# lior1990/hp-vae-gan

Measured on AMD Instinct MI355X. Metric: train iters/sec per pyramid scale, air_balloons 13f@144p, higher is better.
Workload: dtype f32

## Files before the change

### hp-vae-gan_amd/csrc/conv_mfma.hip

```cpp
#include "hpvg_common.h"
#include "hpvg_host.h"
#include "hpvg.h"
#include <stdlib.h>

namespace {

__device__ const float g_zero_word[16] = {0.f, 0.f, 0.f, 0.f, 0.f, 0.f, 0.f, 0.f, 0.f, 0.f, 0.f, 0.f, 0.f, 0.f, 0.f, 0.f};
constexpr long HPVG_ZERO_PLANE_FLOATS = 1L << 18;
__device__ float g_zero_plane[HPVG_ZERO_PLANE_FLOATS];

#ifdef HPVG_TRACE
__device__ unsigned long long g_trace[8192 * 4];
__device__ unsigned long long g_phase[8192 * 4];
#define HPVG_PH(i) { unsigned long long now_ = __builtin_readcyclecounter(); ph_a[i] += now_ - ph_t; ph_t = now_; }
#define HPVG_PH_INIT unsigned long long ph_t = __builtin_readcyclecounter(); unsigned long long ph_a[4] = {0, 0, 0, 0};
#define HPVG_PH_END if (threadIdx.x == 0) { for (int i_ = 0; i_ < 4; ++i_) g_phase[4 * blockIdx.x + i_] = ph_a[i_]; }
#define HPVG_TRACE_BEGIN unsigned long long tr_t0 = wall_clock64(); unsigned long long tr_c0 = __builtin_readcyclecounter();
#define HPVG_TRACE_END                                                              \
  if (threadIdx.x == 0 && blockIdx.x + gridDim.x * (blockIdx.y + gridDim.y * blockIdx.z) < 8192) { \
    unsigned long long* tr = g_trace + 4 * (blockIdx.x + gridDim.x * (blockIdx.y + gridDim.y * blockIdx.z)); \
    tr[0] = tr_t0;                                                                  \
    tr[1] = wall_clock64();                                                         \
    tr[2] = __builtin_amdgcn_s_getreg((31 << 11) | 4);                              \
    tr[3] = (__builtin_amdgcn_s_getreg((31 << 11) | 20) & 0xF) | ((__builtin_readcyclecounter() - tr_c0) << 8); \
// ... 675 lines not shown
      if (n < CO9) {
#pragma unroll
        for (int jj = 0; jj < JB; ++jj)
#pragma unroll
          for (int e = 0; e < 16; ++e) P[n * pitch + GP * grp + JB * ((e & 3) + 8 * (e >> 2) + 4 * half) + jj] = acc[jj][nt][e];
      }
    }
  }
  __syncthreads();

  const int ob = g.ob[band], on = g.on[band];
  const int nout = g.Th * on;
  for (int idx = tid; idx < nout; idx += 256) {
    const int hh = idx / on, cc = idx - hh * on;
    const int gh = h0 + hh, gw = ob + cc;
    if (gh >= a.H) continue;
    const long sp = (long)t * HW + (long)gh * a.W + gw;
    for (int o = 0; o < a.Cout; ++o) {
      float v = 0.f;
#pragma unroll
      for (int dh = 0; dh < 3; ++dh)
#pragma unroll
        for (int dw = 0; dw < 3; ++dw) {
          const int gwt = gw + dw - 1;
          if (gwt >= 0 && gwt < a.W) v += P[(o * 9 + dh * 3 + dw) * pitch + (hh + dh) * RS + (gwt - wsb)];
        }
      if (a.bias) v += a.bias[o];
      if (a.out_lrelu) v = hpvg_lrelu(v);
      a.y[((long)b * a.Cout + o) * a.T * HW + sp] = v;
    }
  }
}

__global__ void conv_pack_narrow_kernel(const float* __restrict__ w, const float* __restrict__ inv_scale, float* __restrict__ wn,
                                        int Cin_k, int Cout_k, int KT, int NT, int ksteps, int transpose_flip, long total) {
  const long idx = (long)blockIdx.x * blockDim.x + threadIdx.x;
  if (idx >= total) return;
  const int lane = idx & 63;
  long r = idx >> 6;
  const int nt = r % NT;
  const int s = (int)(r / NT);
  const int k = (lane >> 5) * ksteps + s;
  const int n = nt * 32 + (lane & 31);
  const int c = k / KT, dt = k - c * KT;
  const int o = n / 9, tap = dt * 9 + (n - o * 9);
  const int taps = KT * 9;
  float val = 0.f;
  if (o < Cout_k && c < Cin_k) {
    if (!transpose_flip) val = w[((long)o * Cin_k + c) * taps + tap];
    else val = w[((long)c * Cout_k + o) * taps + (taps - 1 - tap)];
    if (inv_scale) val *= inv_scale[0];
  }
  wn[idx] = val;
}

__global__ void conv_pack_kernel(const float* __restrict__ w, const float* __restrict__ inv_scale, float* __restrict__ wp,
                                 int Cin_k, int Cout_k, int taps, int CC, int nchunk, int mbtot, int transpose_flip,
                                 long total_direct, long total) {
  const long idx = (long)blockIdx.x * blockDim.x + threadIdx.x;
  if (idx >= total) return;
  if (idx >= total_direct) {
    const long iw = idx - total_direct;
    const long nw1 = ((long)((Cin_k + WINO_CC - 1) / WINO_CC) * (taps / 9) * 3 * 4 + 4) * mbtot * 64 * (WINO_CC / 2);
    float val = iw < nw1 ? wino_pack_value(w, iw, Cin_k, Cout_k, taps / 9, (Cin_k + WINO_CC - 1) / WINO_CC, mbtot, transpose_flip)
                         : wino2_pack_value(w, iw - nw1, Cin_k, Cout_k, (Cin_k + 3) / 4, 2 * ((mbtot + 1) / 2), transpose_flip);
    if (inv_scale) val *= inv_scale[0];
    wp[idx] = val;
    return;
  }
  const int CP = CC / 2;
  long r = idx;
  const int cp = r % CP; r /= CP;
  const int lane = r % 64; r /= 64;
  const int mb = r % mbtot; r /= mbtot;
  const int tap = r % taps; r /= taps;
  const int ch = (int)r;
  float val = 0.f;
  if (ch < nchunk) {
    const int o = mb * 32 + (lane & 31);
    const int c = ch * CC + 2 * cp + (lane >> 5);
    if (o < Cout_k && c < Cin_k) {
      if (!transpose_flip) val = w[((long)o * Cin_k + c) * taps + tap];
      else val = w[((long)c * Cout_k + o) * taps + (taps - 1 - tap)];
      if (inv_scale) val *= inv_scale[0];
    }
  }
  wp[idx] = val;
}

struct PackBatchArgs {
  const float* w[HPVG_PACK_BATCH_MAX];
  float* wp[HPVG_PACK_BATCH_MAX];
  int flip[HPVG_PACK_BATCH_MAX];
};
__global__ void conv_pack_batch_kernel(const PackBatchArgs a, int C, int taps, int CC, int nchunk, int mbtot, long total_direct,
                                       long total) {
  const long idx = (long)blockIdx.x * blockDim.x + threadIdx.x;
  if (idx >= total) return;
  const int it = blockIdx.y;
  const float* __restrict__ w = a.w[it];
  const int transpose_flip = a.flip[it];
  if (idx >= total_direct) {
    const long iw = idx - total_direct;
    const long nw1 = ((long)((C + WINO_CC - 1) / WINO_CC) * (taps / 9) * 3 * 4 + 4) * mbtot * 64 * (WINO_CC / 2);
    a.wp[it][idx] = iw < nw1 ? wino_pack_value(w, iw, C, C, taps / 9, (C + WINO_CC - 1) / WINO_CC, mbtot, transpose_flip)
                             : wino2_pack_value(w, iw - nw1, C, C, (C + 3) / 4, 2 * ((mbtot + 1) / 2), transpose_flip);
    return;
  }
  const int CP = CC / 2;
  long r = idx;
  const int cp = r % CP; r /= CP;
  const int lane = r % 64; r /= 64;
  const int mb = r % mbtot; r /= mbtot;
  const int tap = r % taps; r /= taps;
  const int ch = (int)r;
  float val = 0.f;
  if (ch < nchunk) {
    const int o = mb * 32 + (lane & 31);
    const int c = ch * CC + 2 * cp + (lane >> 5);
    if (o < C && c < C) {
      if (!transpose_flip) val = w[((long)o * C + c) * taps + tap];
      else val = w[((long)c * C + o) * taps + (taps - 1 - tap)];
    }
  }
  a.wp[it][idx] = val;
}

struct CShape { int B, Cin, Cout, T, H, W, KT; };
inline int conv_check(const CShape& c) {
  if (c.B < 1 || c.Cin < 1 || c.Cout < 1 || c.T < 1 || c.H < 1 || c.W < 1) return HPVG_ERR_ARG;
  return c.KT == 1 || c.KT == 3 ? HPVG_OK : HPVG_ERR_UNSUPPORTED;
}

struct CKnobs {
  bool sk_off;
  bool narrow2_off;
  bool w2r;
  bool w2d_off;
  int stagger;
  int only_nb, only_mb, only_ntw;
  int env_wino;
  int wino;
  long min_pos;
  int stg;
  int w2d;
  int gen;
};
CKnobs& cknobs() {
  static CKnobs knobs = [] {
    auto num = [](const char* name, long dflt) { const char* e = getenv(name); return e ? atol(e) : dflt; };
    CKnobs k{};
    k.sk_off = num("HPVG_CONV_SK", 1) == 0;
    k.narrow2_off = num("HPVG_NARROW2", 1) == 0;
    k.w2r = num("HPVG_WINO2R", 1) != 0;
    k.w2d_off = num("HPVG_WINO2D", 1) == 0;
    k.stagger = (int)num("HPVG_WINO_STAGGER", 0);
    k.only_nb = (int)num("HPVG_PLAN_NB", 0);
    k.only_mb = (int)num("HPVG_PLAN_MB", 0);
// ... 509 lines not shown

int pack_weight_launch(const float* w, const float* inv_scale, float* wp, int Cin_layer, int Cout_layer, int KT, int transpose_flip,
                       bool with2d, void* stream) {
  if (!w || !wp || (KT != 1 && KT != 3) || Cin_layer < 1 || Cout_layer < 1) return HPVG_ERR_ARG;
  const int Cin_k = transpose_flip ? Cout_layer : Cin_layer;
  const int Cout_k = transpose_flip ? Cin_layer : Cout_layer;
  const long total = (long)wpack_floats(Cin_k, Cout_k, KT, with2d);
  if (conv_is_narrow(Cin_k, Cout_k)) {
    hipLaunchKernelGGL(conv_pack_narrow_kernel, dim3(hpvg_cdiv(total, 256)), dim3(256), 0, (hipStream_t)stream, w, inv_scale, wp,
                       Cin_k, Cout_k, KT, hpvg_cdiv(9 * Cout_k, 32), hpvg_cdiv(Cin_k * KT, 2), transpose_flip, total);
    return hpvg_launch_status();
  }
  const int CC = conv_cc(Cin_k);
  hipLaunchKernelGGL(conv_pack_kernel, dim3(hpvg_cdiv(total, 256)), dim3(256), 0, (hipStream_t)stream, w, inv_scale, wp, Cin_k, Cout_k,
                     KT * 9, CC, hpvg_cdiv(Cin_k, CC), hpvg_cdiv(Cout_k, 32), transpose_flip, (long)direct_pack_floats(Cin_k, Cout_k, KT),
                     total);
  return hpvg_launch_status();
}

int pack_batch_launch(int n, const float* const* w, float* const* wp, const int* flip, int C, int KT, bool with2d, void* stream) {
  if (n < 1 || n > HPVG_PACK_BATCH_MAX || !w || !wp || !flip || C <= 4 || (KT != 1 && KT != 3)) return HPVG_ERR_ARG;
  PackBatchArgs a;
  for (int i = 0; i < n; ++i) {
    if (!w[i] || !wp[i]) return HPVG_ERR_ARG;
    a.w[i] = w[i]; a.wp[i] = wp[i]; a.flip[i] = flip[i];
  }
  const int CC = conv_cc(C);
  const long total = (long)wpack_floats(C, C, KT, with2d);
  hipLaunchKernelGGL(conv_pack_batch_kernel, dim3(hpvg_cdiv(total, 256), n), dim3(256), 0, (hipStream_t)stream, a, C, KT * 9, CC,
                     hpvg_cdiv(C, CC), hpvg_cdiv(C, 32), (long)direct_pack_floats(C, C, KT), total);
  return hpvg_launch_status();
}

int write_plan(const Plan& p, int out4, int ntiles, int* out) {
  out[0] = p.L; out[1] = p.Tw; out[2] = p.nrange; out[3] = p.ntw; out[4] = out4; out[5] = p.NB; out[6] = p.MB;
  out[7] = p.gridy; out[8] = (int)p.lds; out[9] = ntiles;
  return HPVG_OK;
}

}

extern "C" {

size_t hpvg_conv_wpack_floats(int Cin, int Cout, int KT) { return wpack_floats(Cin, Cout, KT, true); }
size_t hpvg_conv_wpack_floats_for(int Cin, int Cout, int KT, int B, int T, int H, int W) {
  return wpack_floats(Cin, Cout, KT, wants_wino2d({B, Cin, Cout, T, H, W, KT}));
}
int hpvg_conv_wants_wino2d(int B, int Cin, int Cout, int T, int H, int W, int KT) { return wants_wino2d({B, Cin, Cout, T, H, W, KT}) ? 1 : 0; }

int hpvg_conv_pack_weight_f32(const float* w, const float* inv_scale, float* wp, int Cin_layer, int Cout_layer, int KT,
                              int transpose_flip, void* stream) {
  return pack_weight_launch(w, inv_scale, wp, Cin_layer, Cout_layer, KT, transpose_flip, true, stream);
}
int hpvg_conv_pack_weight_for_f32(const float* w, const float* inv_scale, float* wp, int Cin_layer, int Cout_layer, int KT,
                                  int transpose_flip, int B, int T, int H, int W, void* stream) {
  const int Cin_k = transpose_flip ? Cout_layer : Cin_layer, Cout_k = transpose_flip ? Cin_layer : Cout_layer;
  return pack_weight_launch(w, inv_scale, wp, Cin_layer, Cout_layer, KT, transpose_flip, wants_wino2d({B, Cin_k, Cout_k, T, H, W, KT}), stream);
}
int hpvg_conv_pack_weight_batch_f32(int n, const float* const* w, float* const* wp, const int* flip, int C, int KT, void* stream) {
  return pack_batch_launch(n, w, wp, flip, C, KT, true, stream);
}
int hpvg_conv_pack_weight_batch_for_f32(int n, const float* const* w, float* const* wp, const int* flip, int C, int KT, int B, int T,
                                        int H, int W, void* stream) {
  return pack_batch_launch(n, w, wp, flip, C, KT, wants_wino2d({B, C, C, T, H, W, KT}), stream);
}

int hpvg_conv_fwd_f32(const float* x, const float* wp, const float* bias, const float* in_scale, const float* in_shift,
                      int in_lrelu, float* y, int out_lrelu, const float* out_mask, void* ws, size_t ws_bytes, int B, int Cin,
                      int Cout, int T, int H, int W, int KT, void* stream) {
  return conv_fwd_launch({x, wp, bias, in_scale, in_shift, in_lrelu, y, out_lrelu, out_mask, nullptr, nullptr, ws, ws_bytes,
                          {B, Cin, Cout, T, H, W, KT}, (hipStream_t)stream});
}

size_t hpvg_conv_mask_words(int B, int C, int T, int H, int W) { return (size_t)B * T * H * W * hpvg_cdiv(C, 32); }

int hpvg_conv_fwd_bits_f32(const float* x, const float* wp, const float* bias, float* y, int out_lrelu, const unsigned* mask_bits,
                           unsigned* bits_out, void* ws, size_t ws_bytes, int B, int Cin, int Cout, int T, int H, int W, int KT,
                           void* stream) {
  if (conv_is_narrow(Cin, Cout)) return HPVG_ERR_UNSUPPORTED;
  if (mask_bits && bits_out) return HPVG_ERR_UNSUPPORTED;
  return conv_fwd_launch({x, wp, bias, nullptr, nullptr, 0, y, out_lrelu, nullptr, mask_bits, bits_out, ws, ws_bytes,
                          {B, Cin, Cout, T, H, W, KT}, (hipStream_t)stream});
}

int hpvg_conv_fwd_kernel_kind(int B, int Cin, int Cout, int T, int H, int W, int KT) {
  const CShape c{B, Cin, Cout, T, H, W, KT};
  return conv_check(c) == HPVG_OK ? conv_decide_query(c).kind : HPVG_ERR_ARG;
}

size_t hpvg_conv_fwd_ws_bytes(int B, int Cin, int Cout, int T, int H, int W, int KT) {
  const CShape c{B, Cin, Cout, T, H, W, KT};
  if (conv_check(c) != HPVG_OK || conv_is_narrow(Cin, Cout)) return 0;
  const CKnobs& k = cknobs();
  const CPlans& pl = conv_plans(k, c);
  const size_t direct = conv_sk_ws_bytes(c, pl.direct[1]), wino = conv_use_wino(k, c, false) ? conv_sk_ws_bytes(c, pl.wino[1]) : 0;
  return direct > wino ? direct : wino;
}
// ... 54 lines not shown
```

### hp-vae-gan_amd/ops.py

```python
import ctypes
import os

import torch
from torch.autograd import Function
from torch.autograd.function import once_differentiable

from .lib import PACK_BATCH_MAX, SN_BATCH_MAX, call, load, ptr, stream

_ws_cache = {}
_kernel_timer = None


class KernelTimer:

    def __init__(self, match):
        self.match = match
        self.events = []

    def begin(self, desc):
        fam = self.match(desc)
        if not fam:
            return None
        e0 = torch.cuda.Event(enable_timing=True)
        e0.record()
# ... 43 lines not shown
def _scratch(nbytes, device):
    ws = workspace(nbytes, device)
    return ptr(ws), ws.numel()


def _c(t):
    return t if t.is_contiguous() else t.contiguous()


def geom(x):
    if x.dim() == 5:
        B, C, T, H, W = x.shape
    elif x.dim() == 4:
        B, C, H, W = x.shape
        T = 1
    else:
        raise RuntimeError("expected a 4-D or 5-D activation, got %s" % (tuple(x.shape),))
    return B, C, T, H, W


def _kt(w_shape):
    if len(w_shape) == 5:
        if tuple(w_shape[2:]) != (3, 3, 3):
            raise RuntimeError("only 3x3x3 kernels are supported on the MI355X path, got %s" % (tuple(w_shape),))
        return 3
    if len(w_shape) == 4:
        if tuple(w_shape[2:]) != (3, 3):
            raise RuntimeError("only 3x3 kernels are supported on the MI355X path, got %s" % (tuple(w_shape),))
        return 1
    raise RuntimeError("bad weight shape %s" % (tuple(w_shape),))


_pack_cache = {}


def weights_changed():
    _pack_cache.clear()


def _wants_2d(geom_k, cin_k, cout_k, KT):
    if geom_k is None or KT != 3:
        return None if geom_k is None else False
    B, T, H, W = geom_k
    return load().hpvg_conv_wants_wino2d(B, cin_k, cout_k, T, H, W, KT) == 1


def pack_weight(w, flip, geom_k=None):
    w = _c(w)
    Co, Ci = w.shape[0], w.shape[1]
    KT = _kt(w.shape)
    cin_k, cout_k = (Co, Ci) if flip else (Ci, Co)
    has2d = _wants_2d(geom_k, cin_k, cout_k, KT)
    key = (w.data_ptr(), bool(flip), tuple(w.shape))
    hit = _pack_cache.get(key)
    if hit is not None and hit[0] == w._version and hit[1].device == w.device and (hit[3] is None or hit[3] is True or has2d is False):
        return hit[2]
    if geom_k is None:
        n = call("hpvg_conv_wpack_floats", cin_k, cout_k, KT)
        wp = torch.empty(n, dtype=torch.float32, device=w.device)
        call("hpvg_conv_pack_weight_f32", ptr(w), None, ptr(wp), Ci, Co, KT, 1 if flip else 0, stream())
    else:
        B, T, H, W = geom_k
        n = call("hpvg_conv_wpack_floats_for", cin_k, cout_k, KT, B, T, H, W)
        wp = torch.empty(n, dtype=torch.float32, device=w.device)
        call("hpvg_conv_pack_weight_for_f32", ptr(w), None, ptr(wp), Ci, Co, KT, 1 if flip else 0, B, T, H, W, stream())
    _pack_cache[key] = (w._version, w.detach(), wp, has2d)
    return wp


def prepack_weights(ws, flips=(False, True), geom_k=None):
    items = []
    for w in ws:
        if w.dim() < 4 or w.shape[0] != w.shape[1] or w.shape[0] <= 4 or not w.is_contiguous():
            continue
        for f in flips:
            key = (w.data_ptr(), bool(f), tuple(w.shape))
            hit = _pack_cache.get(key)
            if hit is None or hit[0] != w._version:
                items.append((w, bool(f), key))
    if not items:
        return
    shape = tuple(items[0][0].shape)
    items = [it for it in items if tuple(it[0].shape) == shape][:PACK_BATCH_MAX]
    C, KT = shape[0], _kt(shape)
    has2d = _wants_2d(geom_k, C, C, KT)
    if geom_k is None:
        nfl = call("hpvg_conv_wpack_floats", C, C, KT)
    else:
        nfl = call("hpvg_conv_wpack_floats_for", C, C, KT, *geom_k)
    dev = items[0][0].device
    wps = [torch.empty(nfl, dtype=torch.float32, device=dev) for _ in items]
    m = len(items)
    PA, IA = ctypes.c_void_p * m, ctypes.c_int * m
    if geom_k is None:
        call("hpvg_conv_pack_weight_batch_f32", m, PA(*[ptr(it[0]) for it in items]), PA(*[ptr(t) for t in wps]),
             IA(*[1 if it[1] else 0 for it in items]), C, KT, stream())
    else:
        call("hpvg_conv_pack_weight_batch_for_f32", m, PA(*[ptr(it[0]) for it in items]), PA(*[ptr(t) for t in wps]),
             IA(*[1 if it[1] else 0 for it in items]), C, KT, *geom_k, stream())
    for (w, f, key), wp in zip(items, wps):
        _pack_cache[key] = (w._version, w.detach(), wp, has2d)


def conv_fwd_raw(x, w, bias, out_lrelu=False, flip=False, in_affine=None, in_lrelu=False, out_mask=None, mask_bits=None,
                 want_bits=False):
    x = _c(x)
    B, C, T, H, W = geom(x)
    KT = _kt(w.shape)
    Co_l, Ci_l = w.shape[0], w.shape[1]
    cin_k, cout_k = (Co_l, Ci_l) if flip else (Ci_l, Co_l)
    if C != cin_k:
        raise RuntimeError("conv: input has %d channels, weight expects %d" % (C, cin_k))
    wp = pack_weight(w, flip, (B, T, H, W))
    shape = (B, cout_k, T, H, W) if x.dim() == 5 else (B, cout_k, H, W)
    y = torch.empty(shape, dtype=torch.float32, device=x.device)
    sc = sh = None
    if in_affine is not None:
        sc, sh = in_affine
    timed = None
    if _kernel_timer is not None:
        var = "pro" if in_affine is not None else ("mask" if (out_mask is not None or mask_bits is not None) else ("bits" if want_bits else "plain"))
        timed = _kernel_timer.begin({"op": "conv", "Cin": cin_k, "Cout": cout_k, "KT": KT, "flip": flip, "var": var})
    nws = call("hpvg_conv_fwd_ws_bytes", B, cin_k, cout_k, T, H, W, KT)
    ws = _scratch(nws, x.device) if nws else (None, 0)
    if out_mask is not None and tuple(out_mask.shape) != tuple(shape):
        raise RuntimeError("conv: out_mask has shape %s, the output %s" % (tuple(out_mask.shape), tuple(shape)))
    bits = None
    if (mask_bits is not None or want_bits) and cout_k > 4 and in_affine is None:
        if want_bits:
            bits = torch.empty(call("hpvg_conv_mask_words", B, cout_k, T, H, W), dtype=torch.int32, device=x.device)
        if mask_bits is not None and mask_bits.numel() != call("hpvg_conv_mask_words", B, cout_k, T, H, W):
            raise RuntimeError("conv: mask_bits has %d words, the output needs %d" % (mask_bits.numel(), call("hpvg_conv_mask_words", B, cout_k, T, H, W)))
        call("hpvg_conv_fwd_bits_f32", ptr(x), ptr(wp), ptr(bias), ptr(y), 1 if out_lrelu else 0, ptr(mask_bits), ptr(bits), *ws,
             B, cin_k, cout_k, T, H, W, KT, stream())
# ... 888 lines not shown

def host_floats_to_device(values, device):
    vals = [float(v) for v in values]
    if device.type != "cuda":
        return torch.tensor(vals, dtype=torch.float32, device=device)
    if not _pinned_ring:
        _pinned_ring.extend([0, [torch.empty(16, dtype=torch.float32).pin_memory() for _ in range(16)]])
    slot = _pinned_ring[1][_pinned_ring[0] % 16]
    _pinned_ring[0] += 1
    for i, v in enumerate(vals):
        slot[i] = v
    return slot[:len(vals)].to(device, non_blocking=True)


def lerp(a, b, alpha):
    a, b = _c(a.detach()), _c(b.detach())
    out = torch.empty_like(a)
    call("hpvg_lerp_f32", ptr(a), ptr(b), ptr(alpha), ptr(out), a.numel(), stream())
    return out


def sqsum(flat):
    out = _scalar_out(flat.device)
    call("hpvg_sqsum_f32", ptr(flat), ptr(out), *_reduce_ws(flat.device), flat.numel(), stream())
    return out


def clip_scale_(flat_grad, sq, max_norm, coef_out=None):
    call("hpvg_clip_scale_f32", ptr(flat_grad), flat_grad.numel(), ptr(sq), float(max_norm), ptr(coef_out),
         stream())


def adam_step_(p, g, m, v, lr, beta1, beta2, eps, step, step_dev=None):
    weights_changed()
    call("hpvg_adam_step_f32", ptr(p), ptr(g), ptr(m), ptr(v), p.numel(), float(lr), float(beta1), float(beta2),
         float(eps), int(step), ptr(step_dev), stream())


def counter_inc_(counter):
    call("hpvg_counter_inc_i32", ptr(counter), stream())


def video_to_u8(x):
    x = _c(x)
    if x.dtype != torch.float32:
        raise RuntimeError("video_to_u8: fp32 input expected, got %s" % x.dtype)
    if x.dim() == 4:
        B, C, H, W = x.shape
        T = 1
        out = torch.empty(B, H, W, C, dtype=torch.uint8, device=x.device)
    elif x.dim() == 5:
        B, C, T, H, W = x.shape
        out = torch.empty(B, T, H, W, C, dtype=torch.uint8, device=x.device)
    else:
        raise RuntimeError("video_to_u8: expected [B,C,T,H,W] or [B,C,H,W], got %s" % (tuple(x.shape),))
    if out.numel():
        call("hpvg_video_to_u8_f32", ptr(x), ptr(out), B, C, T, H, W, stream())
    return out


def _triple(v, name, op="patch_nn"):
    v = tuple(int(e) for e in v)
    if len(v) != 3:
        raise RuntimeError("%s: %s must have 3 entries (t, h, w), got %d" % (op, name, len(v)))
    return (ctypes.c_int * 3)(*v)


# ... 316 lines not shown
```

### hp-vae-gan_amd/optim.py

```python
import torch

from . import ops

_ALIGN = 64


class ParamArena:

    def __init__(self, module):
        params = list(module.parameters())
        if not params:
            raise ValueError("module has no parameters")
        dev = params[0].device
        offs, total = [], 0
        for p in params:
            offs.append(total)
            total += (p.numel() + _ALIGN - 1) // _ALIGN * _ALIGN
        self.flat = torch.zeros(total, dtype=torch.float32, device=dev)
        self.grad = torch.zeros(total, dtype=torch.float32, device=dev)
        self.range = {}
        with torch.no_grad():
            for p, o in zip(params, offs):
                n = p.numel()
                self.flat[o:o + n].copy_(p.detach().reshape(-1))
                p.data = self.flat[o:o + n].view(p.shape)
                p.grad = self.grad[o:o + n].view(p.shape)
                self.range[id(p)] = (o, n)
        self.params = params
        self.total = total

    def span(self, params):
        rs = sorted(self.range[id(p)] for p in params)
        lo = rs[0][0]
        hi = rs[-1][0] + (rs[-1][1] + _ALIGN - 1) // _ALIGN * _ALIGN
        covered = sum((n + _ALIGN - 1) // _ALIGN * _ALIGN for _, n in rs)
        if covered != hi - lo:
            raise ValueError("parameter group is not contiguous in the arena")
        return lo, hi

    def zero_grad(self):
        self.grad.zero_()
        for p in self.params:
            o, n = self.range[id(p)]
            g = p.grad
            if g is None or g.data_ptr() != self.grad.data_ptr() + 4 * o:
                p.grad = self.grad[o:o + n].view(p.shape)

    def clip_grad_norm_(self, max_norm, info=None):
        sq = ops.sqsum(self.grad)
        ops.clip_scale_(self.grad, sq, max_norm, info)


class BufferArena:

    def __init__(self, module, suffixes=("running_mean", "running_var")):
        items = []
        for mod in module.modules():
            for name, buf in mod._buffers.items():
                if buf is not None and buf.dtype.is_floating_point and name.endswith(tuple(suffixes)):
                    items.append((mod, name, buf))
        self.items = items
        total = sum(b.numel() for _, _, b in items)
# ... 7 lines not shown
                n = buf.numel()
                self.flat[o:o + n].copy_(buf.reshape(-1))
                mod._buffers[name] = self.flat[o:o + n].view(buf.shape)
                o += n


class FlatAdam:

    def __init__(self, arena, groups, betas=(0.5, 0.999), eps=1e-8):
        self.arena = arena
        self.betas = betas
        self.eps = eps
        self.groups = []
        for params, lr in groups:
            params = list(params)
            if not params:
                continue
            lo, hi = arena.span(params)
            layout = [(arena.range[id(p)][0] - lo, p.numel(), tuple(p.shape)) for p in params]
            self.groups.append({"lo": lo, "hi": hi, "lr": lr, "layout": layout,
                                "m": torch.zeros(hi - lo, dtype=torch.float32, device=arena.flat.device),
                                "v": torch.zeros(hi - lo, dtype=torch.float32, device=arena.flat.device)})
        self.t = 0
        self.t_dev = torch.zeros(1, dtype=torch.int32, device=arena.flat.device)

    def step(self):
        self.t += 1
        ops.counter_inc_(self.t_dev)
        for g in self.groups:
            lo, hi = g["lo"], g["hi"]
            ops.adam_step_(self.arena.flat[lo:hi], self.arena.grad[lo:hi], g["m"], g["v"], g["lr"], self.betas[0], self.betas[1],
                           self.eps, self.t, self.t_dev)

    def steps(self):
        return int(self.t_dev.item())

    def state_dict(self):
        t = self.steps()
        state, param_groups, idx = {}, [], 0
        for g in self.groups:
            ids = []
            m, v = g["m"].detach().cpu(), g["v"].detach().cpu()
            for o, n, shape in g["layout"]:
                if t > 0:
                    state[idx] = {"step": torch.tensor(float(t)), "exp_avg": m[o:o + n].view(shape).clone(),
                                  "exp_avg_sq": v[o:o + n].view(shape).clone()}
                ids.append(idx)
                idx += 1
            param_groups.append({"lr": g["lr"], "betas": tuple(self.betas), "eps": self.eps, "weight_decay": 0, "amsgrad": False,
                                 "maximize": False, "foreach": None, "capturable": False, "differentiable": False, "fused": None,
                                 "params": ids})
        return {"state": state, "param_groups": param_groups}
```

### hp-vae-gan_amd/train.py

```python

import torch

from . import ops
from . import optim as hp_optim
from . import utils
from .modules import networks_2d, networks_3d
from .modules.losses import kl_criterion, mse_loss, wgan_mean
from .modules.utils import calc_gradient_penalty


_NODE_TYPES = ["kernel", "memcpy", "memset", "host", "graph", "empty", "wait_event", "event_record", "ext_sem_signal",
               "ext_sem_wait", "mem_alloc", "mem_free", "memcpy_from_symbol", "memcpy_to_symbol", "batch_mem_op", "other"]


def graph_node_census(graph):
    import ctypes
    from .lib import call
    counts = (ctypes.c_int * len(_NODE_TYPES))()
    call("hpvg_graph_node_census", graph.raw_cuda_graph(), counts, len(_NODE_TYPES))
    return {name: int(c) for name, c in zip(_NODE_TYPES, counts)}


def _networks(opt):
    return networks_3d if getattr(opt, 'dims', 3) == 3 else networks_2d
# ... 6 lines not shown
        if opt.vae_levels < opt.scale_idx + 1:
            depth = min(opt.train_depth, len(body) - opt.vae_levels + 1)
            blocks = list(body[-depth:])
            groups += [(b.parameters(), opt.lr_g * (opt.lr_scale ** (len(blocks) - 1 - i))) for i, b in enumerate(blocks)]
        else:
            lr0 = opt.lr_g * (opt.lr_scale ** opt.scale_idx)
            groups += [(netG.encode.parameters(), lr0), (netG.decoder.parameters(), lr0)]
            blocks = list(body[-opt.train_depth:])
            groups += [(b.parameters(), opt.lr_g * (opt.lr_scale ** (len(blocks) - 1 - i))) for i, b in enumerate(blocks)]
    else:
        if len(body) < opt.train_depth:
            lr0 = opt.lr_g * (opt.lr_scale ** opt.scale_idx)
            groups += [(netG.encode.parameters(), lr0), (netG.decoder.parameters(), lr0)]
            groups += [(b.parameters(), opt.lr_g * (opt.lr_scale ** (len(body) - 1 - i))) for i, b in enumerate(body)]
        else:
            blocks = list(body[-opt.train_depth:])
            groups += [(b.parameters(), opt.lr_g * (opt.lr_scale ** (len(blocks) - 1 - i))) for i, b in enumerate(blocks)]
    return groups


def _capture_iteration(trainer, run, nets):
    ops.pin_workspaces()
    side = torch.cuda.Stream()
    side.wait_stream(torch.cuda.current_stream())
    with torch.cuda.stream(side):
        warm = run()
    torch.cuda.current_stream().wait_stream(side)
    trainer.warmup_out = warm
    it = trainer.iteration
    graph = torch.cuda.CUDAGraph(keep_graph=True)
    bns = [m for net in nets if net is not None for m in net.modules() if hasattr(m, 'pending_batches')]
    before = [m.pending_batches for m in bns]
    host = _host_state(trainer)
    ops.weights_changed()
    ok = False
    try:
        with torch.cuda.graph(graph):
            trainer._g_out = run()
        ops.weights_changed()
        trainer.graph_nodes = graph_node_census(graph)
        bad = {k: v for k, v in trainer.graph_nodes.items() if k not in ("kernel", "empty", "event_record", "wait_event") and v}
        if bad:
            raise GraphCaptureRefused("the captured iteration holds non-kernel graph nodes %s (of %s): refusing to replay it"
                                      % (bad, trainer.graph_nodes))
        graph.instantiate()
        trainer._graph = graph
        trainer._graph_bn = [(m, m.pending_batches - b) for m, b in zip(bns, before) if m.pending_batches != b]
        ok = True
    finally:
        for m, b in zip(bns, before):
            m.pending_batches = b
        trainer.iteration = it
        if not ok:
            trainer._graph = None
            trainer._g_out = None
            _restore_host_state(trainer, host)
    return warm


class GraphCaptureRefused(RuntimeError):
    """the captured iteration cannot be replayed safely (non-kernel graph nodes); the trainer is left in its eager state"""


def _host_state(trainer):
    st = {"opt": [(o, o.t) for o in (getattr(trainer, n, None) for n in ("optimizerG", "optimizerD")) if o is not None and hasattr(o, "t")]}
    dev = getattr(getattr(trainer, "opt", None), "device", None)
    try:
        rs = ops._rng(torch.device(dev)) if dev is not None and torch.device(dev).type == "cuda" else None
    except Exception:
        rs = None
    st["rng"] = (rs, rs.call) if rs is not None else None
    return st


def _restore_host_state(trainer, st):
    for o, t in st["opt"]:
        o.t = t
    if st["rng"] is not None:
        st["rng"][0].call = st["rng"][1]


def _replay_iteration(trainer):
    trainer._graph.replay()
    ops.weights_changed()
    for m, d in trainer._graph_bn:
        m.pending_batches += d
    trainer.iteration += 1
    return trainer._g_out


class StageTrainer:

    def __init__(self, opt, netG, netD=None):
        self.opt = opt
        self.netG = netG
        self.dims = getattr(opt, 'dims', 3)
        nets = _networks(opt)
        self.is_gan = opt.vae_levels < opt.scale_idx + 1
        self.netD = None
        if self.is_gan:
            self.netD = netD if netD is not None else getattr(nets, opt.discriminator)(opt).to(opt.device)
            self.arenaD = hp_optim.ParamArena(self.netD)
            self.optimizerD = hp_optim.FlatAdam(self.arenaD, [(self.netD.parameters(), opt.lr_d)], betas=(opt.beta1, 0.999))
        self.arenaG = hp_optim.ParamArena(netG)
        self.optimizerG = hp_optim.FlatAdam(self.arenaG, generator_param_groups(opt, netG), betas=(opt.beta1, 0.999))
        level0 = utils.images.level_shape_3d(0, opt) if self.dims == 3 else utils.images.level_shape_2d(0, opt)
        opt.Z_init_size = [opt.batch_size, opt.latent_dim, *level0]
        self.iteration = 0
        self.clip_info = torch.zeros(2, dtype=torch.float32, device=opt.device)
        self.last = {}
        self.after_d_step = None
        self.alpha_source = getattr(opt, "alpha_source", None)
        self.loss_log = None

    def calibrate_noise_amp(self, real, real_zero):
        opt = self.opt
        if opt.const_amp:
# ... 262 lines not shown
```

### include/hpvg.h

```cpp
#ifndef HPVG_H
#define HPVG_H
#include <stddef.h>
#ifdef __cplusplus
extern "C" {
#endif

#define HPVG_OK 0
#define HPVG_ERR_ARG (-1)
#define HPVG_ERR_WORKSPACE (-2)
#define HPVG_ERR_UNSUPPORTED (-3)
#define HPVG_ERR_LAUNCH (-4)

size_t hpvg_conv_wpack_floats(int Cin, int Cout, int KT);
int hpvg_conv_pack_weight_f32(const float* w, const float* inv_scale, float* wp, int Cin_layer, int Cout_layer, int KT,
                              int transpose_flip, void* stream);
#define HPVG_PACK_BATCH_MAX 16
int hpvg_conv_pack_weight_batch_f32(int n, const float* const* w, float* const* wp, const int* flip, int C, int KT, void* stream);
size_t hpvg_conv_wpack_floats_for(int Cin, int Cout, int KT, int B, int T, int H, int W);
int hpvg_conv_wants_wino2d(int B, int Cin, int Cout, int T, int H, int W, int KT);
int hpvg_conv_pack_weight_for_f32(const float* w, const float* inv_scale, float* wp, int Cin_layer, int Cout_layer, int KT,
                                  int transpose_flip, int B, int T, int H, int W, void* stream);
int hpvg_conv_pack_weight_batch_for_f32(int n, const float* const* w, float* const* wp, const int* flip, int C, int KT, int B, int T,
                                        int H, int W, void* stream);
size_t hpvg_conv_fwd_ws_bytes(int B, int Cin, int Cout, int T, int H, int W, int KT);
int hpvg_conv_fwd_f32(const float* x, const float* wp, const float* bias, const float* in_scale, const float* in_shift,
                      int in_lrelu, float* y, int out_lrelu, const float* out_mask, void* ws, size_t ws_bytes, int B, int Cin,
                      int Cout, int T, int H, int W, int KT, void* stream);
size_t hpvg_conv_mask_words(int B, int C, int T, int H, int W);
int hpvg_conv_fwd_bits_f32(const float* x, const float* wp, const float* bias, float* y, int out_lrelu, const unsigned* mask_bits,
                           unsigned* bits_out, void* ws, size_t ws_bytes, int B, int Cin, int Cout, int T, int H, int W, int KT,
                           void* stream);
int hpvg_conv_fwd_plan(int B, int Cin, int Cout, int T, int H, int W, int KT, int* out10);
int hpvg_conv_fwd_kernel_kind(int B, int Cin, int Cout, int T, int H, int W, int KT);
int hpvg_conv_wino_config(int mode, long min_positions);
int hpvg_conv_wino_plan(int B, int Cin, int Cout, int T, int H, int W, int KT, int* out10);
int hpvg_conv_narrow_plan(int B, int Cin, int Cout, int T, int H, int W, int KT, int* out55);
size_t hpvg_conv_bwd_weight_ws_bytes(int B, int Cin, int Cout, int T, int H, int W, int KT);
int hpvg_conv_bwd_weight_f32(const float* dy, const float* x, const float* in_scale, const float* in_shift, int in_lrelu,
                             float* dw, int accumulate, void* ws, size_t ws_bytes, int B, int Cin, int Cout, int T, int H,
                             int W, int KT, void* stream);
int hpvg_conv_bwd_weight_plan(int B, int Cin, int Cout, int T, int H, int W, int KT, int* out10);
int hpvg_conv_bwd_weight_kernel_kind(int B, int Cin, int Cout, int T, int H, int W, int KT);
int hpvg_conv_bwd_weight_wino_config(int mode);
int hpvg_conv_bwd_weight_fuses_bias(int B, int Cin, int Cout, int T, int H, int W, int KT);
int hpvg_conv_bwd_weight_bias_f32(const float* dy, const float* x, float* dw, int accumulate, float* db, int accumulate_db, void* ws,
                                  size_t ws_bytes, int B, int Cin, int Cout, int T, int H, int W, int KT, void* stream);
int hpvg_conv_bwd_weight_wino_plan(int B, int Cin, int Cout, int T, int H, int W, int KT, int* out10);
int hpvg_conv_bwd_weight_wino2_plan(int B, int Cin, int Cout, int T, int H, int W, int KT, int* out11);
size_t hpvg_channel_sum_ws_bytes(int C);
int hpvg_channel_sum_f32(const float* x, float* out, int accumulate, void* ws, size_t ws_bytes, int B, int C, long S,
                         void* stream);

size_t hpvg_bn_ws_bytes(int C);
int hpvg_bn_train_stats_f32(const float* x, const float* gamma, const float* beta, float* running_mean, float* running_var,
                            float momentum, float eps, float* mean, float* invstd, float* scale, float* shift, void* ws,
                            size_t ws_bytes, int B, int C, long S, void* stream);
// ... 142 lines not shown
```

Measured before the change: 31.87.

## Keep weight packs across steps and batch repacks of mixed-shape weights in one launch

Replaces the global pack-cache clear after every optimizer step with range-based invalidation, so only the packs of parameters whose optimizer ranges were stepped are dropped. Dropped packs are queued and later repacked together through a new list kernel that handles heterogeneous shapes, narrow and wide layouts in a single launch. During graph replay, packs created outside the graph are refreshed when their weight version has changed. The aim is to cut the number of per-iteration pack kernel launches and avoid repacking unchanged weights, at the cost of more complex cache bookkeeping and a risk of using stale packs if the version tracking misses an update.

Result: no change. 32.08, median of 6 (+0.7%).

```diff
diff --git a/hp-vae-gan_amd/csrc/conv_mfma.hip b/hp-vae-gan_amd/csrc/conv_mfma.hip
--- a/hp-vae-gan_amd/csrc/conv_mfma.hip
+++ b/hp-vae-gan_amd/csrc/conv_mfma.hip
@@ -731,10 +731,8 @@
   }
 }
 
-__global__ void conv_pack_narrow_kernel(const float* __restrict__ w, const float* __restrict__ inv_scale, float* __restrict__ wn,
-                                        int Cin_k, int Cout_k, int KT, int NT, int ksteps, int transpose_flip, long total) {
-  const long idx = (long)blockIdx.x * blockDim.x + threadIdx.x;
-  if (idx >= total) return;
+__device__ inline float narrow_pack_value(const float* __restrict__ w, const float* __restrict__ inv_scale, long idx, int Cin_k,
+                                          int Cout_k, int KT, int NT, int ksteps, int transpose_flip) {
   const int lane = idx & 63;
   long r = idx >> 6;
   const int nt = r % NT;
@@ -750,22 +748,24 @@
     else val = w[((long)c * Cout_k + o) * taps + (taps - 1 - tap)];
     if (inv_scale) val *= inv_scale[0];
   }
-  wn[idx] = val;
-}
-
-__global__ void conv_pack_kernel(const float* __restrict__ w, const float* __restrict__ inv_scale, float* __restrict__ wp,
-                                 int Cin_k, int Cout_k, int taps, int CC, int nchunk, int mbtot, int transpose_flip,
-                                 long total_direct, long total) {
+  return val;
+}
+__global__ void conv_pack_narrow_kernel(const float* __restrict__ w, const float* __restrict__ inv_scale, float* __restrict__ wn,
+                                        int Cin_k, int Cout_k, int KT, int NT, int ksteps, int transpose_flip, long total) {
   const long idx = (long)blockIdx.x * blockDim.x + threadIdx.x;
   if (idx >= total) return;
+  wn[idx] = narrow_pack_value(w, inv_scale, idx, Cin_k, Cout_k, KT, NT, ksteps, transpose_flip);
+}
+
+__device__ inline float wide_pack_value(const float* __restrict__ w, const float* __restrict__ inv_scale, long idx, int Cin_k,
+                                        int Cout_k, int taps, int CC, int nchunk, int mbtot, int transpose_flip, long total_direct) {
   if (idx >= total_direct) {
     const long iw = idx - total_direct;
     const long nw1 = ((long)((Cin_k + WINO_CC - 1) / WINO_CC) * (taps / 9) * 3 * 4 + 4) * mbtot * 64 * (WINO_CC / 2);
     float val = iw < nw1 ? wino_pack_value(w, iw, Cin_k, Cout_k, taps / 9, (Cin_k + WINO_CC - 1) / WINO_CC, mbtot, transpose_flip)
                          : wino2_pack_value(w, iw - nw1, Cin_k, Cout_k, (Cin_k + 3) / 4, 2 * ((mbtot + 1) / 2), transpose_flip);
     if (inv_scale) val *= inv_scale[0];
-    wp[idx] = val;
-    return;
+    return val;
   }
   const int CP = CC / 2;
   long r = idx;
@@ -784,7 +784,14 @@
       if (inv_scale) val *= inv_scale[0];
     }
   }
-  wp[idx] = val;
+  return val;
+}
+__global__ void conv_pack_kernel(const float* __restrict__ w, const float* __restrict__ inv_scale, float* __restrict__ wp,
+                                 int Cin_k, int Cout_k, int taps, int CC, int nchunk, int mbtot, int transpose_flip,
+                                 long total_direct, long total) {
+  const long idx = (long)blockIdx.x * blockDim.x + threadIdx.x;
+  if (idx >= total) return;
+  wp[idx] = wide_pack_value(w, inv_scale, idx, Cin_k, Cout_k, taps, CC, nchunk, mbtot, transpose_flip, total_direct);
 }
 
 struct PackBatchArgs {
@@ -797,32 +804,29 @@
   const long idx = (long)blockIdx.x * blockDim.x + threadIdx.x;
   if (idx >= total) return;
   const int it = blockIdx.y;
-  const float* __restrict__ w = a.w[it];
-  const int transpose_flip = a.flip[it];
-  if (idx >= total_direct) {
-    const long iw = idx - total_direct;
-    const long nw1 = ((long)((C + WINO_CC - 1) / WINO_CC) * (taps / 9) * 3 * 4 + 4) * mbtot * 64 * (WINO_CC / 2);
-    a.wp[it][idx] = iw < nw1 ? wino_pack_value(w, iw, C, C, taps / 9, (C + WINO_CC - 1) / WINO_CC, mbtot, transpose_flip)
-                             : wino2_pack_value(w, iw - nw1, C, C, (C + 3) / 4, 2 * ((mbtot + 1) / 2), transpose_flip);
-    return;
-  }
-  const int CP = CC / 2;
-  long r = idx;
-  const int cp = r % CP; r /= CP;
-  const int lane = r % 64; r /= 64;
-  const int mb = r % mbtot; r /= mbtot;
-  const int tap = r % taps; r /= taps;
-  const int ch = (int)r;
-  float val = 0.f;
-  if (ch < nchunk) {
-    const int o = mb * 32 + (lane & 31);
-    const int c = ch * CC + 2 * cp + (lane >> 5);
-    if (o < C && c < C) {
-      if (!transpose_flip) val = w[((long)o * C + c) * taps + tap];
-      else val = w[((long)c * C + o) * taps + (taps - 1 - tap)];
-    }
-  }
-  a.wp[it][idx] = val;
+  a.wp[it][idx] = wide_pack_value(a.w[it], nullptr, idx, C, C, taps, CC, nchunk, mbtot, a.flip[it], total_direct);
+}
+
+struct PackListItem {
+  const float* w;
+  float* wp;
+  long total_direct, total;
+  int Cin_k, Cout_k, KT, flip, narrow;
+  int a, b, c;
+};
+struct PackListArgs {
+  PackListItem item[HPVG_PACK_BATCH_MAX];
+  int block0[HPVG_PACK_BATCH_MAX + 1];
+  int n;
+};
+__global__ __launch_bounds__(256) void conv_pack_list_kernel(const PackListArgs a) {
+  int it = 0;
+  while (it + 1 < a.n && (int)blockIdx.x >= a.block0[it + 1]) ++it;
+  const PackListItem& p = a.item[it];
+  const long idx = (long)(blockIdx.x - a.block0[it]) * 256 + threadIdx.x;
+  if (idx >= p.total) return;
+  p.wp[idx] = p.narrow ? narrow_pack_value(p.w, nullptr, idx, p.Cin_k, p.Cout_k, p.KT, p.a, p.b, p.flip)
+                       : wide_pack_value(p.w, nullptr, idx, p.Cin_k, p.Cout_k, p.KT * 9, p.a, p.b, p.c, p.flip, p.total_direct);
 }
 
 struct CShape { int B, Cin, Cout, T, H, W, KT; };
@@ -1398,6 +1402,35 @@
   return hpvg_launch_status();
 }
 
+int pack_list_launch(int n, const float* const* w, float* const* wp, const int* desc, void* stream) {
+  if (n < 1 || n > HPVG_PACK_BATCH_MAX || !w || !wp || !desc) return HPVG_ERR_ARG;
+  PackListArgs a;
+  a.n = n;
+  long blocks = 0;
+  for (int i = 0; i < n; ++i) {
+    const int* d = desc + 8 * i;
+    const int Cin_layer = d[0], Cout_layer = d[1], KT = d[2], flip = d[3] ? 1 : 0;
+    if (!w[i] || !wp[i] || (KT != 1 && KT != 3) || Cin_layer < 1 || Cout_layer < 1) return HPVG_ERR_ARG;
+    const int Cin_k = flip ? Cout_layer : Cin_layer, Cout_k = flip ? Cin_layer : Cout_layer;
+    const CShape c{d[4], Cin_k, Cout_k, d[5], d[6], d[7], KT};
+    if (conv_check(c) != HPVG_OK) return HPVG_ERR_ARG;
+    PackListItem& p = a.item[i];
+    p.w = w[i]; p.wp = wp[i];
+    p.Cin_k = Cin_k; p.Cout_k = Cout_k; p.KT = KT; p.flip = flip;
+    p.narrow = conv_is_narrow(Cin_k, Cout_k) ? 1 : 0;
+    p.total = (long)wpack_floats(Cin_k, Cout_k, KT, wants_wino2d(c));
+    p.total_direct = p.narrow ? 0 : (long)direct_pack_floats(Cin_k, Cout_k, KT);
+    if (p.narrow) { p.a = hpvg_cdiv(9 * Cout_k, 32); p.b = hpvg_cdiv(Cin_k * KT, 2); p.c = 0; }
+    else { p.a = conv_cc(Cin_k); p.b = hpvg_cdiv(Cin_k, p.a); p.c = hpvg_cdiv(Cout_k, 32); }
+    a.block0[i] = (int)blocks;
+    blocks += hpvg_cdiv(p.total, 256);
+    if (blocks > 0x7fffffffL) return HPVG_ERR_ARG;
+  }
+  for (int i = n; i <= HPVG_PACK_BATCH_MAX; ++i) a.block0[i] = (int)blocks;
+  hipLaunchKernelGGL(conv_pack_list_kernel, dim3((unsigned)blocks), dim3(256), 0, (hipStream_t)stream, a);
+  return hpvg_launch_status();
+}
+
 int write_plan(const Plan& p, int out4, int ntiles, int* out) {
   out[0] = p.L; out[1] = p.Tw; out[2] = p.nrange; out[3] = p.ntw; out[4] = out4; out[5] = p.NB; out[6] = p.MB;
   out[7] = p.gridy; out[8] = (int)p.lds; out[9] = ntiles;
@@ -1429,6 +1462,10 @@
 int hpvg_conv_pack_weight_batch_for_f32(int n, const float* const* w, float* const* wp, const int* flip, int C, int KT, int B, int T,
                                         int H, int W, void* stream) {
   return pack_batch_launch(n, w, wp, flip, C, KT, wants_wino2d({B, C, C, T, H, W, KT}), stream);
+}
+
+int hpvg_conv_pack_weight_list_for_f32(int n, const float* const* w, float* const* wp, const int* desc, void* stream) {
+  return pack_list_launch(n, w, wp, desc, stream);
 }
 
 int hpvg_conv_fwd_f32(const float* x, const float* wp, const float* bias, const float* in_scale, const float* in_shift,
diff --git a/hp-vae-gan_amd/ops.py b/hp-vae-gan_amd/ops.py
--- a/hp-vae-gan_amd/ops.py
+++ b/hp-vae-gan_amd/ops.py
@@ -99,10 +99,59 @@
 
 
 _pack_cache = {}
-
-
-def weights_changed():
-    _pack_cache.clear()
+_pack_pending = {}
+_pack_epoch = [0]
+_PACK_KEEP = os.environ.get("HPVG_PACK_KEEP", "1") != "0"
+
+
+class _Pack:
+    __slots__ = ("version", "w", "flip", "wp", "has2d", "geom_k", "keep", "used", "epoch")
+
+    def __init__(self, w, flip, wp, has2d, geom_k, keep):
+        self.version, self.w, self.flip, self.wp, self.has2d, self.geom_k, self.keep = w._version, w.detach(), flip, wp, has2d, geom_k, keep
+        self.used = False
+        _pack_epoch[0] += 1
+        self.epoch = _pack_epoch[0]
+
+
+def weights_changed(ranges=None):
+    if ranges is None or not _PACK_KEEP:
+        _pack_cache.clear()
+        _pack_pending.clear()
+        return
+    lo, hi = (min(r[0] for r in ranges), max(r[1] for r in ranges)) if ranges else (0, 0)
+    for key in [k for k, e in _pack_cache.items() if not e.keep or (lo <= k[0] < hi and any(a <= k[0] < b for a, b in ranges))]:
+        e = _pack_cache.pop(key)
+        if e.keep and e.used and e.geom_k is not None:
+            _pack_pending[key] = (e.w, key[1], e.geom_k)
+
+
+def pack_mark():
+    return _pack_epoch[0]
+
+
+def drop_packs_since(mark):
+    for key in [k for k, e in _pack_cache.items() if e.epoch > mark]:
+        del _pack_cache[key]
+
+
+def pack_entries():
+    return list(_pack_cache.values())
+
+
+def refresh_packs(entries):
+    for e in entries:
+        if e.w._version != e.version:
+            _pack_into(e.w, e.flip, e.geom_k, e.wp)
+            e.version = e.w._version
+
+
+def _pack_into(w, flip, geom_k, wp):
+    Co, Ci, KT = w.shape[0], w.shape[1], _kt(w.shape)
+    if geom_k is None:
+        call("hpvg_conv_pack_weight_f32", ptr(w), None, ptr(wp), Ci, Co, KT, 1 if flip else 0, stream())
+    else:
+        call("hpvg_conv_pack_weight_for_f32", ptr(w), None, ptr(wp), Ci, Co, KT, 1 if flip else 0, *geom_k, stream())
 
 
 def _wants_2d(geom_k, cin_k, cout_k, KT):
@@ -110,6 +159,36 @@
         return None if geom_k is None else False
     B, T, H, W = geom_k
     return load().hpvg_conv_wants_wino2d(B, cin_k, cout_k, T, H, W, KT) == 1
+
+
+def _pack_list(items):
+    for i in range(0, len(items), PACK_BATCH_MAX):
+        part = items[i:i + PACK_BATCH_MAX]
+        m = len(part)
+        desc, wps, has2ds = [], [], []
+        for w, f, geom_k, _ in part:
+            Co, Ci, KT = w.shape[0], w.shape[1], _kt(w.shape)
+            cin_k, cout_k = (Co, Ci) if f else (Ci, Co)
+            desc += [Ci, Co, KT, 1 if f else 0, *geom_k]
+            wps.append(torch.empty(call("hpvg_conv_wpack_floats_for", cin_k, cout_k, KT, *geom_k), dtype=torch.float32, device=w.device))
+            has2ds.append(_wants_2d(geom_k, cin_k, cout_k, KT))
+        PA = ctypes.c_void_p * m
+        call("hpvg_conv_pack_weight_list_for_f32", m, PA(*[ptr(it[0]) for it in part]), PA(*[ptr(t) for t in wps]),
+             (ctypes.c_int * (8 * m))(*desc), stream())
+        for (w, f, geom_k, keep), wp, has2d in zip(part, wps, has2ds):
+            key = (w.data_ptr(), bool(f), tuple(w.shape))
+            _pack_pending.pop(key, None)
+            _pack_cache[key] = _Pack(w, bool(f), wp, has2d, geom_k, keep)
+
+
+def _pending_items(room):
+    if len(_pack_pending) > room:
+        return []
+    return [(w, f, geom_k, True) for w, f, geom_k in _pack_pending.values()]
+
+
+def _keeps(w):
+    return _PACK_KEEP and isinstance(w, torch.nn.Parameter)
 
 
 def pack_weight(w, flip, geom_k=None):
@@ -120,53 +199,50 @@
     has2d = _wants_2d(geom_k, cin_k, cout_k, KT)
     key = (w.data_ptr(), bool(flip), tuple(w.shape))
     hit = _pack_cache.get(key)
-    if hit is not None and hit[0] == w._version and hit[1].device == w.device and (hit[3] is None or hit[3] is True or has2d is False):
-        return hit[2]
-    if geom_k is None:
-        n = call("hpvg_conv_wpack_floats", cin_k, cout_k, KT)
-        wp = torch.empty(n, dtype=torch.float32, device=w.device)
-        call("hpvg_conv_pack_weight_f32", ptr(w), None, ptr(wp), Ci, Co, KT, 1 if flip else 0, stream())
-    else:
-        B, T, H, W = geom_k
-        n = call("hpvg_conv_wpack_floats_for", cin_k, cout_k, KT, B, T, H, W)
-        wp = torch.empty(n, dtype=torch.float32, device=w.device)
-        call("hpvg_conv_pack_weight_for_f32", ptr(w), None, ptr(wp), Ci, Co, KT, 1 if flip else 0, B, T, H, W, stream())
-    _pack_cache[key] = (w._version, w.detach(), wp, has2d)
+    if hit is not None and hit.version == w._version and hit.w.device == w.device and (hit.has2d is None or hit.has2d is True or has2d is False):
+        hit.used = True
+        return hit.wp
+    if geom_k is not None and _pack_pending.pop(key, None) is not None:
+        _pack_list([(w, flip, geom_k, True)] + _pending_items(len(_pack_pending)))
+        hit = _pack_cache[key]
+        hit.used = True
+        return hit.wp
+    n = call("hpvg_conv_wpack_floats", cin_k, cout_k, KT) if geom_k is None else call("hpvg_conv_wpack_floats_for", cin_k, cout_k, KT, *geom_k)
+    wp = torch.empty(n, dtype=torch.float32, device=w.device)
+    _pack_into(w, flip, geom_k, wp)
+    hit = _pack_cache[key] = _Pack(w, bool(flip), wp, has2d, geom_k, _keeps(w))
+    hit.used = True
     return wp
 
 
 def prepack_weights(ws, flips=(False, True), geom_k=None):
     items = []
     for w in ws:
-        if w.dim() < 4 or w.shape[0] != w.shape[1] or w.shape[0] <= 4 or not w.is_contiguous():
+        if w.dim() < 4 or not w.is_contiguous() or (geom_k is None and (w.shape[0] != w.shape[1] or w.shape[0] <= 4)):
             continue
         for f in flips:
             key = (w.data_ptr(), bool(f), tuple(w.shape))
             hit = _pack_cache.get(key)
-            if hit is None or hit[0] != w._version:
+            if hit is None or hit.version != w._version:
                 items.append((w, bool(f), key))
     if not items:
+        return
+    if geom_k is not None:
+        room = -len(items) % PACK_BATCH_MAX
+        _pack_list([(w, f, geom_k, _keeps(w)) for w, f, _ in items] + _pending_items(room))
         return
     shape = tuple(items[0][0].shape)
     items = [it for it in items if tuple(it[0].shape) == shape][:PACK_BATCH_MAX]
     C, KT = shape[0], _kt(shape)
-    has2d = _wants_2d(geom_k, C, C, KT)
-    if geom_k is None:
-        nfl = call("hpvg_conv_wpack_floats", C, C, KT)
-    else:
-        nfl = call("hpvg_conv_wpack_floats_for", C, C, KT, *geom_k)
+    nfl = call("hpvg_conv_wpack_floats", C, C, KT)
     dev = items[0][0].device
     wps = [torch.empty(nfl, dtype=torch.float32, device=dev) for _ in items]
     m = len(items)
     PA, IA = ctypes.c_void_p * m, ctypes.c_int * m
-    if geom_k is None:
-        call("hpvg_conv_pack_weight_batch_f32", m, PA(*[ptr(it[0]) for it in items]), PA(*[ptr(t) for t in wps]),
-             IA(*[1 if it[1] else 0 for it in items]), C, KT, stream())
-    else:
-        call("hpvg_conv_pack_weight_batch_for_f32", m, PA(*[ptr(it[0]) for it in items]), PA(*[ptr(t) for t in wps]),
-             IA(*[1 if it[1] else 0 for it in items]), C, KT, *geom_k, stream())
+    call("hpvg_conv_pack_weight_batch_f32", m, PA(*[ptr(it[0]) for it in items]), PA(*[ptr(t) for t in wps]),
+         IA(*[1 if it[1] else 0 for it in items]), C, KT, stream())
     for (w, f, key), wp in zip(items, wps):
-        _pack_cache[key] = (w._version, w.detach(), wp, has2d)
+        _pack_cache[key] = _Pack(w, f, wp, None, None, False)
 
 
 def conv_fwd_raw(x, w, bias, out_lrelu=False, flip=False, in_affine=None, in_lrelu=False, out_mask=None, mask_bits=None,
@@ -1121,7 +1197,7 @@
 
 
 def adam_step_(p, g, m, v, lr, beta1, beta2, eps, step, step_dev=None):
-    weights_changed()
+    weights_changed([(p.data_ptr(), p.data_ptr() + 4 * p.numel())])
     call("hpvg_adam_step_f32", ptr(p), ptr(g), ptr(m), ptr(v), p.numel(), float(lr), float(beta1), float(beta2),
          float(eps), int(step), ptr(step_dev), stream())
 
diff --git a/hp-vae-gan_amd/optim.py b/hp-vae-gan_amd/optim.py
--- a/hp-vae-gan_amd/optim.py
+++ b/hp-vae-gan_amd/optim.py
@@ -28,6 +28,7 @@
                 self.range[id(p)] = (o, n)
         self.params = params
         self.total = total
+        ops.weights_changed()
 
     def span(self, params):
         rs = sorted(self.range[id(p)] for p in params)
@@ -101,6 +102,10 @@
             ops.adam_step_(self.arena.flat[lo:hi], self.arena.grad[lo:hi], g["m"], g["v"], g["lr"], self.betas[0], self.betas[1],
                            self.eps, self.t, self.t_dev)
 
+    def ranges(self):
+        base = self.arena.flat.data_ptr()
+        return [(base + 4 * g["lo"], base + 4 * g["hi"]) for g in self.groups]
+
     def steps(self):
         return int(self.t_dev.item())
 
diff --git a/hp-vae-gan_amd/train.py b/hp-vae-gan_amd/train.py
--- a/hp-vae-gan_amd/train.py
+++ b/hp-vae-gan_amd/train.py
@@ -62,12 +62,16 @@
     bns = [m for net in nets if net is not None for m in net.modules() if hasattr(m, 'pending_batches')]
     before = [m.pending_batches for m in bns]
     host = _host_state(trainer)
-    ops.weights_changed()
+    ops.weights_changed(_stepped_ranges(trainer))
+    trainer._graph_packs = ops.pack_entries()
+    mark = ops.pack_mark()
     ok = False
     try:
-        with torch.cuda.graph(graph):
-            trainer._g_out = run()
-        ops.weights_changed()
+        try:
+            with torch.cuda.graph(graph):
+                trainer._g_out = run()
+        finally:
+            ops.drop_packs_since(mark)
         trainer.graph_nodes = graph_node_census(graph)
         bad = {k: v for k, v in trainer.graph_nodes.items() if k not in ("kernel", "empty", "event_record", "wait_event") and v}
         if bad:
@@ -84,6 +88,7 @@
         if not ok:
             trainer._graph = None
             trainer._g_out = None
+            trainer._graph_packs = None
             _restore_host_state(trainer, host)
     return warm
 
@@ -110,9 +115,14 @@
         st["rng"][0].call = st["rng"][1]
 
 
+def _stepped_ranges(trainer):
+    return [r for n in ("optimizerG", "optimizerD") if hasattr(getattr(trainer, n, None), "ranges") for r in getattr(trainer, n).ranges()]
+
+
 def _replay_iteration(trainer):
+    ops.refresh_packs(trainer._graph_packs)
     trainer._graph.replay()
-    ops.weights_changed()
+    ops.weights_changed(_stepped_ranges(trainer))
     for m, d in trainer._graph_bn:
         m.pending_batches += d
     trainer.iteration += 1
diff --git a/include/hpvg.h b/include/hpvg.h
--- a/include/hpvg.h
+++ b/include/hpvg.h
@@ -22,6 +22,7 @@
                                   int transpose_flip, int B, int T, int H, int W, void* stream);
 int hpvg_conv_pack_weight_batch_for_f32(int n, const float* const* w, float* const* wp, const int* flip, int C, int KT, int B, int T,
                                         int H, int W, void* stream);
+int hpvg_conv_pack_weight_list_for_f32(int n, const float* const* w, float* const* wp, const int* desc, void* stream);
 size_t hpvg_conv_fwd_ws_bytes(int B, int Cin, int Cout, int T, int H, int W, int KT);
 int hpvg_conv_fwd_f32(const float* x, const float* wp, const float* bias, const float* in_scale, const float* in_shift,
                       int in_lrelu, float* y, int out_lrelu, const float* out_mask, void* ws, size_t ws_bytes, int B, int Cin,
```
